# byteowlz/kokorox

Measured on AMD Instinct MI355X. Metric: real-time factor (audio-s/wall-s), 24 kHz, batch=64, higher is better.
Workload: dtype f32 in / out, f32 accumulate; products on split operands: f16f8 (a_hi b_hi on f16 MFMAs, the cross terms a_lo b_hi + a_hi b_lo of the 7 / 11-tap convs on e4m3 scaled MFMAs: ~17 significant bits per product; every other conv f16x3: ~22) -- wider than the bf16 BASELINE configs[2] names, inside the 1e-; 1 GPU; batch=64/GPU synthetic 128-phoneme utterances (T=130), durations pinned 3,3,3,4 -> F=422 frames = 10.55 s each, noise on, inputs in HBM; batch_per_gpu=64, frames=422, parallelism=utterance-sharded x1, one-time weight broadcast

## Files before the change

### kokorox_amd/build.py

```python
from __future__ import annotations

import os
import subprocess
import sys

HERE = os.path.dirname(os.path.abspath(__file__))
CSRC = os.path.join(HERE, "csrc")
LIB_DIR = os.path.join(HERE, "lib")
LIB_PATH = os.path.join(LIB_DIR, "libkokorox_hip.so")
TEST_LIB_PATH = os.path.join(LIB_DIR, "libkokorox_hip_test.so")
TEST_SOURCES = ["test_hooks.hip"]
SOURCES = ["conv_mfma.hip", "conv_f16x3.hip", "conv_f16x3_da.hip", "conv_f16x3_da_p1.hip", "conv_f16x3_da_w2.hip", "conv_f16x3_da_s16.hip", "conv_f16x3_da_f8.hip", "conv_f16x3_da_pre.hip", "conv_f16x3_pre.hip", "conv_f16x3_dapn.hip", "conv_f16x3_dag.hip", "kernels_misc.hip", "model.hip", "api.hip", "dispatcher.hip", "onnx_import.cpp"]
HEADERS = ["kx_common.h", "kx_error.h", "conv_epilogue.h", "conv_f16x3_common.h"]
_PUB = os.path.join("..", "..", "include", "kokorox_hip.h")
_PUB_TEST = os.path.join("..", "..", "include", "kokorox_hip_test.h")
EXTRA_DEPS = {"model.hip": ["onnx_import.h", "model.h", _PUB], "api.hip": ["model.h", "kx_handle.h", "api_guard.h", _PUB],
              "dispatcher.hip": ["model.h", "kx_handle.h", "dispatcher_core.h", _PUB],
              "test_hooks.hip": ["model.h", "kx_handle.h", "api_guard.h", _PUB, _PUB_TEST], "onnx_import.cpp": ["onnx_import.h"], "conv_f16x3_da_p1.hip": ["conv_f16x3_da.hip"], "conv_f16x3_da_w2.hip": ["conv_f16x3_da.hip"], "conv_f16x3_da_s16.hip": ["conv_f16x3_da.hip"], "conv_f16x3_da_f8.hip": ["conv_f16x3_da.hip"], "conv_f16x3_da_pre.hip": ["conv_f16x3_da.hip"]}
FLAGS = ["-O3", "--offload-arch=gfx950", "-fPIC", "-std=c++17", "-Wall", "-Wno-unused-result"]


def _hipcc() -> str:
    for cand in (os.environ.get("HIPCC"), "/opt/rocm/bin/hipcc", "hipcc"):
        if cand and (os.path.isabs(cand) and os.path.exists(cand) or not os.path.isabs(cand)):
            return cand
    return "hipcc"


def _newer(target: str, deps) -> bool:
    if not os.path.exists(target):
        return False
    t = os.path.getmtime(target)
    return all(os.path.getmtime(d) <= t for d in deps)


LAST_BUILD = {"compiled": [], "reused": [], "linked": False}


def build_library(force: bool = False, verbose: bool = False) -> str:
    LAST_BUILD["compiled"], LAST_BUILD["reused"], LAST_BUILD["linked"] = [], [], False
    os.makedirs(LIB_DIR, exist_ok=True)
    hdrs = [os.path.join(CSRC, h) for h in HEADERS]
    objs, test_objs, jobs = [], [], []
    for src in SOURCES + TEST_SOURCES:
        s = os.path.join(CSRC, src)
        o = os.path.join(LIB_DIR, os.path.splitext(src)[0] + ".o")
        (test_objs if src in TEST_SOURCES else objs).append(o)
        if force or not _newer(o, [s] + hdrs + [os.path.join(CSRC, d) for d in EXTRA_DEPS.get(src, [])]):
            flags = [f for f in FLAGS if not f.startswith("--offload-arch")] if src.endswith(".cpp") else FLAGS
            jobs.append([_hipcc(), *flags, "-c", s, "-o", o])
            LAST_BUILD["compiled"].append(src)
# ... 30 lines not shown
```

### kokorox_amd/csrc/conv_f16x3.hip

```cpp
#include "conv_f16x3_common.h"

namespace kx {

template <int BM, int BN, int WM, int WN, int ACT, int TK, bool PF, int VT>
__global__ __launch_bounds__(WM * WN * 64, (WM * WN == 8) ? 4 : ((BM / WM / 32) * (BN / WN / 32) > 6 ? 2 : 3))
void conv1d_f16x3_kernel(const ConvArgs a) {
    constexpr int MT = BM / WM / 32;
    constexpr int NT = BN / WN / 32;
    constexpr int NWV = WM * WN;
    static_assert((NWV == 4 || NWV == 8) && MT >= 1 && NT >= 1, "4 or 8 waves per workgroup");
    static_assert(VT == 1 || (VT <= TK && PF), "virtual taps need TK >= VT and the prefetching build");
    extern __shared__ __attribute__((aligned(16))) unsigned char smem16[];

    const int tid = threadIdx.x;
    const int lane = tid & 63;
    const int wave = __builtin_amdgcn_readfirstlane(tid >> 6);
    const int wm = wave / WN, wn = wave % WN;
    const int r = lane & 31, h = lane >> 5;
    const int b = blockIdx.z, ct = blockIdx.y;
    int tile_x = blockIdx.x;
    if (a.xcd_swizzle && gridDim.x >= 16) {
        const int nx = gridDim.x;
        const int off = (int)(((long)nx * (blockIdx.y + (long)gridDim.y * blockIdx.z)) & 7);
        const int cls = (blockIdx.x + off) & 7;
// ... 328 lines not shown

template <int BM, int BN, int WM, int WN, int ACT, int TK>
static void launch_inst16_act(const ConvArgs& a, int B, int max_cols, hipStream_t s) {
    static const int pf_env = env_int("KX_PF", 1);
    const int XW = (BN - 1) * a.stride + (a.K - 1) * a.dil + 1;
    if (pf_env && a.stride == 1 && XW <= BN + 128)
        launch_inst16_pf<BM, BN, WM, WN, ACT, TK, true>(a, B, max_cols, s);
    else
        launch_inst16_pf<BM, BN, WM, WN, ACT, TK, false>(a, B, max_cols, s);
}

template <int BM, int BN, int WM, int WN, int TK>
static void launch_inst16_tk(const ConvArgs& a, int B, int max_cols, hipStream_t s) {
    if (a.act == ACT_SNAKE)
        launch_inst16_act<BM, BN, WM, WN, ACT_SNAKE, TK>(a, B, max_cols, s);
    else if (a.act == ACT_LEAKY)
        launch_inst16_act<BM, BN, WM, WN, ACT_LEAKY, TK>(a, B, max_cols, s);
    else
        launch_inst16_act<BM, BN, WM, WN, ACT_NONE, TK>(a, B, max_cols, s);
}

template <int BM, int BN, int WM, int WN>
static void launch_inst16(const ConvArgs& a, int B, int max_cols, hipStream_t s) {
#ifndef KX_TK
#define KX_TK 3
#endif
    launch_inst16_tk<BM, BN, WM, WN, KX_TK>(a, B, max_cols, s);
}

void conv16_pick_tile(int BM, int max_cols, int B, int Cout, int K, int dil, int stride, int* bn, int* wn, int ws_force, bool stats,
                      int act, int n_chunks16, int pmode) {
    static const int force = env_int("KX_BN", 0);
    if (ws_force != 1 && act >= 0 && conv16_da_s16_shape(BM, K, dil, stride, act, n_chunks16, false, pmode)) {
        const bool small = (long)((max_cols + 255) / 256) * ((Cout + 127) / 128) * B < 256 && ws_force != 2;
        *bn = small ? 128 : 192;
        *wn = small ? 2 : 3;
        return;
    }
    if (ws_force == 2 && conv16_da_eligible(BM, K, dil, stride, 0)) {
        *bn = 256; *wn = 2;
        return;
    }
    if (BM != 128) {
        *bn = 256; *wn = 4;
    } else if ((force == 128 || max_cols <= 160) && !stats) {
        *bn = 128; *wn = 2;
    } else if ((long)((max_cols + 255) / 256) * ((Cout + 127) / 128) * B < 256 && force != 256) {
        *bn = 128; *wn = 1;
    } else {
        *bn = 256; *wn = 2;
    }
}

int conv16_flat_bn(const ConvArgs& a, int BM, int B, int max_cols) {
    static const int on = env_int("KX_FLAT", 1);
    if (!on || BM != 128 || B < 2 || max_cols <= 0 || a.merge_T > 0 || a.ws_force == 1 || a.stamps) return 0;
    if (a.K == 1 && a.stride == 1 && !a.stat_part && !a.in_up2 && a.n_chunks16 >= 3 && a.act != ACT_SNAKE) return 0;
    int bn, wn;
    conv16_pick_tile(BM, max_cols, B, a.Cout, a.K, a.dil, a.stride, &bn, &wn, a.ws_force, a.stat_part != nullptr, a.act, a.n_chunks16,
                     conv16_pmode(a));
    if (conv16_da_s16_shape(BM, a.K, a.dil, a.stride, a.act, a.n_chunks16, a.merge_T > 0, conv16_pmode(a))) return bn;
    if (bn == 128 && wn == 1) return conv16_use_da(BM, a.K, a.dil, a.stride, a.merge_T > 0) ? 128 : 0;
    if (bn == 128) return 0;
    return conv16_use_da(BM, a.K, a.dil, a.stride, a.merge_T > 0) ? 256 : 0;
}

void launch_conv1d_f16x3(const ConvArgs& a, int BM, int B, int max_cols, hipStream_t s) {
#ifdef KX_ONLY_MAIN
    launch_inst16_pf<128, 256, 2, 2, ACT_SNAKE, 3, true>(a, B, max_cols, s);
    return;
#else
    KX_REQUIRE(a.n_chunks16 == (a.Cin + CK16 - 1) / CK16 && a.w16 != nullptr, "conv1d f16x3: weights not packed");
// ... 215 lines not shown
```

### kokorox_amd/csrc/conv_f16x3_da.hip

```cpp
#include "conv_f16x3_common.h"
#include <type_traits>


#ifndef KX_F8_RAW_AUX
#define KX_F8_RAW_AUX 0
#endif
#ifndef KX_F8_HWCOS
#define KX_F8_HWCOS 1
#endif

namespace kx {

template <int I, int N, class F>
__device__ __forceinline__ void static_for(F&& f) {
    if constexpr (I < N) {
        f(std::integral_constant<int, I>{});
        static_for<I + 1, N>(f);
    }
}

#if !defined(KX_DA_P1) && !defined(KX_DA_W2) && !defined(KX_DA_S16) && !defined(KX_DA_PRE)
bool conv16_da_eligible(int BM, int K, int dil, int stride, int merged) {
    return BM == 128 && stride == 1 && !merged && (K - 1) * dil + 256 <= 384;
}
// ... 14 lines not shown
    }
    static constexpr int age(int kind, int id) {
        int n = 0, result = -1;
        int st_h[3 * KT + 8] = {}, st_x[3 * NC + 8] = {};
        for (int sc = 0; sc < 2; ++sc) {
            for (int p = 0; p < KT; ++p) {
                if (p == HS) n += RAW;
                if (sc == 1) {
                    if (kind == 0 && p == id) result = n - st_h[KT + p];
                    if (kind == 1 && cross_of(p) == id) result = n - st_x[NC + id];
                }
                n += 2;
                st_h[p + RH <= KT - 1 ? sc * KT + p + RH : (sc + 1) * KT + p % RH] = n;
                const int c = cross_of(p);
                if (c >= 0) {
                    n += 4;
                    st_x[sc * NC + c + RC] = n;
                }
            }
            n += RAW;
        }
        return result < 63 ? result : 63;
    }
    static constexpr int cum(int NB, int first, int n) {
        int t = 0;
        for (int r = 0; r < n; ++r) t += cross_of((first + r) / NB) >= 0 ? 3 : 1;
        return t;
    }
    static constexpr int hu_before(int NB, int NA, int HU, int first, int I0, int rel) {
        return rel > I0 ? ((cum(NB, first, rel) - cum(NB, first, I0)) * HU) / (cum(NB, first, NA) - cum(NB, first, I0)) : 0;
    }
};

template <int ACT, int KT, int NTT, bool P1, bool W2 = false, bool S16 = false, bool PRE = false, bool BF = false, bool F8 = false>
__global__ __launch_bounds__(256, (NTT == 8 || S16) ? 2 : 3) void conv1d_f16x3_da_kernel(const ConvArgs a) {
    static_assert(!BF || P1, "BF: a form of the reduced-precision kernels only");
    static_assert(!F8 || (S16 && KT % 4 == 3), "F8: a form of the S16 loop; tap groups of four with one padding slot");
    constexpr bool HWC = F8 && KX_F8_HWCOS;
    static_assert(!PRE || (!P1 && !S16 && ACT == ACT_NONE), "PRE: the activation lives in the image; f16x3 forms on 32x32x16 only");
    static_assert(!W2 || (KT >= 3 && (KT & 1) && NTT == 8), "W2: odd compile-time tap counts on the 256-column tile");
    static_assert(!S16 || (KT >= 3 && (KT & 1) && !P1 && !W2), "S16: odd compile-time tap counts, three MFMAs per product, 4 x 1 waves");
    static_assert(NTT == 8 || NTT == 4 || (NTT == 6 && S16), "tile widths: 256, 128, and 192 columns in the S16 form");
    constexpr int BM = 128, NT = NTT, BN = 32 * NT;
    constexpr bool W64 = KT > 0;
    constexpr bool SPLIT = W64 && BN % 128 == 0;
    constexpr int NJF = W64 ? (SPLIT ? BN / 128 : (BN + 64) / 128) : (BN + 128) / 128;
    constexpr int NJ = NJF + (SPLIT ? 1 : 0);
    constexpr int HU = 8 * NJF + (SPLIT ? 4 : 0);
    constexpr int XWp = W64 ? BN + 64 : BN + 128;
    static_assert(!W64 || SPLIT || (BN + 64) % 128 == 0, "the window is whole 64-column blocks in pairs, or ends in a split block");
    constexpr int XBUF = 4 * XWp;
    constexpr int tap_units = 4 * BM;
    extern __shared__ __attribute__((aligned(16))) unsigned char smem16[];
    uint4* Xs = reinterpret_cast<uint4*>(smem16);

    const int tid = threadIdx.x;
    const int lane = tid & 63;
    const int wave = __builtin_amdgcn_readfirstlane(tid >> 6);
    const int r = lane & 31, h = lane >> 5;
    auto pack_pair = [](float v0, float v1, unsigned& hi_pk, unsigned& lo_pk) __attribute__((always_inline)) {
        if constexpr (BF) {
            auto rne = [](float x) __attribute__((always_inline)) {
                unsigned u = __builtin_bit_cast(unsigned, x);
                u += 0x7fffu + ((u >> 16) & 1u);
                return u >> 16;
            };
            hi_pk = rne(v0) | (rne(v1) << 16);
            lo_pk = 0u;
        } else if constexpr (F8) {
            split_pair_f8(v0, v1, hi_pk, lo_pk);
        } else {
            split_pair(v0, v1, hi_pk, lo_pk);
        }
    };
    auto act_in = [](float y, float slope, float al, float ial) __attribute__((always_inline)) {
        if constexpr (ACT == ACT_SNAKE && HWC) {
            const float u = (al * y) * 0.318309886183790672f;
            return __builtin_fmaf(ial, __builtin_fmaf(-0.5f, __builtin_amdgcn_cosf(u), 0.5f), y);
        } else {
// ... 22 lines not shown
            const int mid = (lo + hi) >> 1;
            if (a.tile_prefix[mid] <= gt) lo = mid;
            else hi = mid;
        }
        b = __builtin_amdgcn_readfirstlane(lo);
        tile_x = gt - a.tile_prefix[b];
    } else {
        const int nx = gridDim.x, ny = gridDim.y, N = nx * ny;
        const int l = blockIdx.x + nx * blockIdx.y;
        int lp = l;
        if (a.xcd_swizzle && N >= 16) {
            const int off = (int)(((long)N * blockIdx.z) & 7);
            const int cls = (l + off) & 7;
            int start = 0;
            for (int c = 0; c < cls; ++c) {
                const int first = (c - off) & 7;
                start += first < N ? (N - first + 7) >> 3 : 0;
            }
            lp = start + (l >> 3);
        }
        if (a.xcd_swizzle) {
            tile_x = lp / ny;
            ct = lp - tile_x * ny;
        }
    }
    if (a.dephase_cycles > 0) {
        const unsigned gl = blockIdx.x + gridDim.x * (blockIdx.y + gridDim.y * blockIdx.z);
        const bool late = a.dephase_mode == 1 ? (gl < 512u && ((gl >> 3) & 1u)) : (gl >= 256u && gl < 512u);
        if (late) {
            const unsigned long long t_end = __builtin_amdgcn_s_memtime() + (unsigned long long)a.dephase_cycles;
            while (__builtin_amdgcn_s_memtime() < t_end) __builtin_amdgcn_s_sleep(64);
        }
    }
    const int t0 = tile_x * BN;
    const int Lin = a.in_len.lens[b] * a.in_len.mul + a.in_len.add;
    const int Lout = a.out_len.lens[b] * a.out_len.mul + a.out_len.add;
    const int ncols = (a.store == ST_UPSCATTER) ? (Lin + 1) : Lout;
    if (t0 >= ncols) return;

    const int K = KT > 0 ? KT : a.K, dil = a.dil;
    const int n_chunks = a.n_chunks16;
    const int n_steps = n_chunks * K;
    const float* xb = a.x + (long)b * a.x_bs;
    const int p0 = t0 - a.pad;
    const bool has_norm = a.nmean != nullptr;
    const int up2 = a.in_up2;
    const int Lsrc = up2 ? ((Lin + 1) >> 1) : Lin;

    f32x16 acc[1][NT];
#pragma unroll
    for (int j = 0; j < NT; ++j)
#pragma unroll
        for (int e = 0; e < 16; ++e) acc[0][j][e] = 0.f;
    constexpr int NB16 = S16 ? 2 * NT : 1;
    f32x4v acc16[2][NB16];
#pragma unroll
    for (int i = 0; i < 2; ++i)
#pragma unroll
        for (int j = 0; j < NB16; ++j) acc16[i][j] = f32x4v{0.f, 0.f, 0.f, 0.f};

    const int g = wave & 1, jb = wave >> 1;
    float raw[NJ][8];
    float praw[4];
    int xoff[NJ];
    unsigned okmask = 0;
    auto blk_col = [&](int j) __attribute__((always_inline)) { return (SPLIT && j == NJF) ? 64 * 2 * NJF : 64 * (jb + 2 * j); };
#pragma unroll
    for (int j = 0; j < NJ; ++j) {
        const int p = p0 + lane + blk_col(j);
        okmask |= (p >= 0 && p < Lin) ? (1u << j) : 0u;
        int pi = up2 ? (p >> 1) : p;
        pi = pi < 0 ? 0 : (pi >= Lsrc ? Lsrc - 1 : pi);
        xoff[j] = pi;
    }
    using u32x4 = __attribute__((ext_vector_type(4))) unsigned;
    constexpr int NLD = PRE ? (4 * XWp) / 256 : 1;
    static_assert(!PRE || (4 * XWp) % 256 == 0, "PRE: whole rounds of 256 lanes");
    u32x4 rawq[NLD];
    unsigned qoff[NLD];
    unsigned okq = 0;
    const buf_rsrc xq = make_buf(PRE ? reinterpret_cast<const char*>(a.x16) + (long)b * a.x16_bs : reinterpret_cast<const char*>(a.x));
    const unsigned chunk_bytes = PRE ? 64u * (unsigned)a.x16_ld : 0u;
    const buf_rsrc xrow = make_buf(xb);
    if constexpr (PRE) {
#pragma unroll
        for (int i = 0; i < NLD; ++i) {
            const int idx = tid + 256 * i, plane = idx / XWp, u = idx - plane * XWp;
            const int p = p0 + u;
            okq |= (p >= 0 && p < Lin) ? (1u << i) : 0u;
            const int pc = p < 0 ? 0 : (p >= Lin ? Lin - 1 : p);
            qoff[i] = 16u * (unsigned)(plane * a.x16_ld + pc);
        }
    }
    const int cmax_in = a.Cin - 1;
    const float* nm_src = has_norm ? a.nmean + (long)b * a.n_bs : xb;
    const float* ns_src = has_norm ? a.nscale + (long)b * a.n_bs : xb;
    const float* nh_src = has_norm ? a.nshift + (long)b * a.n_bs : xb;
    auto load_params = [&](int ch, float (&pv)[4]) __attribute__((always_inline)) {
        const int c = ch * CK16 + g * 8 + (lane & 7);
// ... 290 lines not shown
#define F8_WAIT_T1 if (a.stamps) acc_wait += __builtin_amdgcn_s_memrealtime() - tb0;
#else
#define F8_BAR_T0
#define F8_BAR_T1
#define F8_WAIT_T1
#endif
#ifndef KX_F8_RH
#define KX_F8_RH ((KT - 1) % 3 != 0 ? 3 : 4)
#endif
#ifndef KX_F8_RC
#define KX_F8_RC (NT == 6 ? 1 : 2)
#endif
        constexpr int RH = KX_F8_RH, RC = KX_F8_RC;
        using FS = F8Sched<KT, RH, RC, raw_ops>;
        constexpr int NG = FS::NG, NC = FS::NC;
        static_assert(RH <= KT && (KT - 1) % RH != 0 && NC % RC == 0, "f16f8: static ring slots");
        static_assert(2 * (NG - 1) <= HS && KT - 1 - 2 * (NG - 1) >= HS && (HS & 1), "f16f8: cross groups inside their buffer's phase");
        const int n_super = n_chunks >> 1;
        const int d_norm = tau16 ? dil : 0, d_str = tau16 ? XBUF - (KT - 1) * dil : 0;
        int d_x2 = tau16 ? 2 * dil : 0;
        int d_xl = tau16 ? 0 : dil;
        using v8i = __attribute__((ext_vector_type(8))) int;
        u32x4 hs[RH][2], xs[RC][4];
        auto make_srd = [](const void* base) __attribute__((always_inline)) {
            const unsigned long long pa = (unsigned long long)base;
            u32x4 srd;
            srd[0] = __builtin_amdgcn_readfirstlane((unsigned)pa);
            srd[1] = __builtin_amdgcn_readfirstlane((unsigned)(pa >> 32) & 0xffffu);
            srd[2] = 0xffffffffu;
            srd[3] = 0x00020000u;
            return srd;
        };
        const u32x4 srd_h = make_srd(a.w16), srd_x = make_srd(a.w8x);
        const unsigned voff_h = 16u * (unsigned)(tau16 * tap_units + h16 * BM + wave * 32 + r16);
        const unsigned voff_x = 16u * (unsigned)((lane >> 4) * 256 + wave * 32 + r16);
        const unsigned tile_h = (unsigned)__builtin_amdgcn_readfirstlane(ct * n_steps), tile_x8 = (unsigned)__builtin_amdgcn_readfirstlane(ct * n_chunks * NG);
        auto load_H = [&](int s0, u32x4 (&xh)[2]) __attribute__((always_inline)) {
            const unsigned so = (tile_h + (unsigned)__builtin_amdgcn_readfirstlane(s0 < n_steps - 2 ? s0 : n_steps - 2)) * (16u * tap_units);
            asm volatile("buffer_load_dwordx4 %0, %1, %2, %3 offen" : "=v"(xh[0]) : "v"(voff_h), "s"(srd_h), "s"(so) : "memory");
            asm volatile("buffer_load_dwordx4 %0, %1, %2, %3 offen offset:256" : "=v"(xh[1]) : "v"(voff_h), "s"(srd_h), "s"(so) : "memory");
        };
        auto load_X = [&](int chunk, const int m, u32x4 (&x)[4]) __attribute__((always_inline)) {
            const unsigned so = (tile_x8 + (unsigned)__builtin_amdgcn_readfirstlane(chunk < n_chunks ? chunk : n_chunks - 1) * NG + m) * 16384u;
            asm volatile("buffer_load_dwordx4 %0, %1, %2, %3 offen" : "=v"(x[0]) : "v"(voff_x), "s"(srd_x), "s"(so) : "memory");
            asm volatile("buffer_load_dwordx4 %0, %1, %2, %3 offen offset:2048" : "=v"(x[1]) : "v"(voff_x), "s"(srd_x), "s"(so) : "memory");
            asm volatile("buffer_load_dwordx4 %0, %1, %2, %3 offen offset:256" : "=v"(x[2]) : "v"(voff_x), "s"(srd_x), "s"(so) : "memory");
            asm volatile("buffer_load_dwordx4 %0, %1, %2, %3 offen offset:2304" : "=v"(x[3]) : "v"(voff_x), "s"(srd_x), "s"(so) : "memory");
        };
        static_for<0, RH>([&](auto qc) __attribute__((always_inline)) { load_H(2 * decltype(qc)::value, hs[decltype(qc)::value]); });
        static_for<0, RC>([&](auto qc) __attribute__((always_inline)) {
            constexpr int c = decltype(qc)::value;
            load_X(c >= NG ? 1 : 0, c >= NG ? c - NG : c, xs[c]);
        });
        asm volatile("s_waitcnt vmcnt(0)" ::: "memory");
        int xl_it = h16 * XWp + r16;
        int dil_it = dil;
        half8 fh[2];
        v8i fx[2];
        auto load_blk_h = [&](const int p, const int nb, half8& fhx) __attribute__((always_inline)) {
            const int f0 = 2 * p, b0 = f0 >= KT ? 1 : 0, tp = f0 - b0 * KT;
            const uint4* xt = Xs + (xl_it + b0 * XBUF + tp * dil_it + (f0 == KT - 1 ? d_str : d_norm) + nb * 16);
            fhx = *reinterpret_cast<const half8*>(xt);
        };
        auto load_blk_x = [&](const int c, const int nb, v8i& fxx) __attribute__((always_inline)) {
            const int b0 = c >= NG ? 1 : 0, m = c - b0 * NG;
            const uint4* xt = Xs + (xl_it + 2 * XWp + b0 * XBUF + 4 * m * dil_it + d_x2 + nb * 16);
            const uint4 u0 = *xt, u1 = *(xt + (m == NG - 1 ? d_xl : dil_it));
            fxx = v8i{(int)u0.x, (int)u0.y, (int)u0.z, (int)u0.w, (int)u1.x, (int)u1.y, (int)u1.z, (int)u1.w};
        };
// ... 550 lines not shown
                        for (int c = 0; c < 8; ++c) asm volatile("" ::"v"(raw[j][c]));
                } else if (!(a.dbg & 1))
                    stage_from_raw(Xs + (cur ^ 1) * XBUF, ch);
                asm volatile("s_waitcnt lgkmcnt(0)\n\ts_barrier" ::: "memory");
                cur ^= 1;
                if (ch + 1 < n_chunks && !(a.dbg & (1 | 2048))) {
                    load_raw(ch + 1);
                    age += raw_ops;
                    o1 += raw_ops;
                    o2 += raw_ops;
                }
                load_tile(0, 0, fh[(E0 + NT) % 3], fl[(E0 + NT) % 3]);
                load_tile(0, 1, fh[(E0 + NT + 1) % 3], fl[(E0 + NT + 1) % 3]);
            }
        }
    };
    for (int s3 = 0; s3 < n_steps; s3 += 3) {
        step(0, ah0, al0, age0, age1, age2, s3);
        if (s3 + 1 < n_steps) step(NT % 3, ah1, al1, age1, age2, age0, s3 + 1);
        if (s3 + 2 < n_steps) step((2 * NT) % 3, ah2, al2, age2, age0, age1, s3 + 2);
    }
    }
    asm volatile("s_waitcnt vmcnt(0)" ::: "memory");
#ifdef KX_DA_STAMPS
    if (a.stamps) st2 = __builtin_amdgcn_s_memrealtime();
#endif
    if (a.dbg & 8) return;
    asm volatile("s_waitcnt lgkmcnt(0)\n\ts_barrier" ::: "memory");
    float2* stat_scr = reinterpret_cast<float2*>(smem16) + wave * (32 * 33);
    float* wide_scr = reinterpret_cast<float*>(stat_scr);
    if constexpr (S16) {
        static_for<0, NT / 2>([&](auto gc) __attribute__((always_inline)) {
            constexpr int g2 = decltype(gc)::value;
            conv_store_group16<EPI_ROWS, NB16, 2, NT == 6>(a, acc16, 4 * g2, a.w_unscale, b, ct * BM + wave * 32, t0 + 64 * g2, lane, ncols, Lout,
                                                  tile_x * (NT / 2) + g2, stat_scr, wide_scr);
        });
    } else if constexpr (W2) {
        conv_store_group<EPI_ROWS, true>(a, *reinterpret_cast<f32x16(*)[1][4]>(&acc[0][0]), a.w_unscale, b, ct * BM + wr2 * 64, t0 + 128 * wc2, r,
                                   h, ncols, Lout, tile_x * 2 + wc2, stat_scr, wide_scr);
        conv_store_group<EPI_ROWS, true>(a, *reinterpret_cast<f32x16(*)[1][4]>(&acc[0][4]), a.w_unscale, b, ct * BM + wr2 * 64 + 32, t0 + 128 * wc2,
                                   r, h, ncols, Lout, tile_x * 2 + wc2, stat_scr, wide_scr);
    } else if constexpr (NT == 8) {
        conv_store_group<EPI_ROWS>(a, *reinterpret_cast<f32x16(*)[1][4]>(&acc[0][0]), a.w_unscale, b, ct * BM + wave * 32, t0, r, h,
                                   ncols, Lout, tile_x * 2, stat_scr, wide_scr);
        conv_store_group<EPI_ROWS>(a, *reinterpret_cast<f32x16(*)[1][4]>(&acc[0][4]), a.w_unscale, b, ct * BM + wave * 32, t0 + 128, r,
                                   h, ncols, Lout, tile_x * 2 + 1, stat_scr, wide_scr);
    } else {
        conv_store_group<EPI_ROWS>(a, acc, a.w_unscale, b, ct * BM + wave * 32, t0, r, h, ncols, Lout, tile_x, stat_scr, wide_scr);
    }
#ifdef KX_DA_STAMPS
    if (a.stamps && tid == 0) {
        const unsigned lin = blockIdx.x + gridDim.x * (blockIdx.y + gridDim.y * blockIdx.z);
        unsigned long long* o = a.stamps + (unsigned long long)lin * 8;
        o[0] = st0; o[1] = st1; o[2] = st2;
        __builtin_amdgcn_s_waitcnt(0);
        o[3] = __builtin_amdgcn_s_memrealtime();
        o[4] = __builtin_amdgcn_s_getreg(63492);
        o[5] = __builtin_readcyclecounter() - cyc0;
        o[6] = F8 ? acc_wait : __builtin_amdgcn_s_getreg(63508);
        o[7] = acc_bar;
    }
#endif
}

#ifdef KX_DA_P1
constexpr bool DA_P1 = true;
#else
constexpr bool DA_P1 = false;
#endif

#ifdef KX_DA_W2
constexpr bool DA_W2 = true;
#else
constexpr bool DA_W2 = false;
#endif

#ifdef KX_DA_S16
constexpr bool DA_S16 = true;
#else
constexpr bool DA_S16 = false;
#endif

#ifdef KX_DA_F8
constexpr bool DA_F8 = true;
#else
constexpr bool DA_F8 = false;
#endif

template <int ACT, int KT, int NTT, bool W2X = DA_W2, bool PREX = false, bool BFX = false>
static void launch_da_inst(const ConvArgs& a, int B, int max_cols, hipStream_t s) {
    auto kern = conv1d_f16x3_da_kernel<ACT, KT, NTT, DA_P1, W2X, DA_S16, PREX, BFX, DA_F8>;
    constexpr int BN = 32 * NTT;
    constexpr size_t lds_x = 16 * (size_t)2 * 4 * (BN + 128), lds_scr = 4 * 32 * 33 * sizeof(float2);
    constexpr size_t lds = lds_x > lds_scr ? lds_x : lds_scr;
    dim3 grid((max_cols + BN - 1) / BN, (a.Cout + 127) / 128, B);
    KX_REQUIRE(grid.x > 0 && grid.y > 0 && grid.y < 65536 && B > 0 && B < 65536, "conv1d f16x3 da: bad grid");
    if (a.tile_prefix) {
        KX_REQUIRE(a.flat_ny == (int)grid.y && a.flat_B == B && a.flat_bn_host == BN && a.flat_tiles_host > 0 &&
                       (long)a.flat_tiles_host * grid.y < (1L << 30),
                   "conv1d f16x3 da: flat tile list does not match the launch");
        grid = dim3((unsigned)a.flat_tiles_host * grid.y, 1, 1);
    }
    hipLaunchKernelGGL(kern, grid, dim3(256), lds, s, a);
    KX_HIP(hipGetLastError());
}

#ifdef KX_DA_PRE
void launch_conv1d_f16x3_da_pre(const ConvArgs& a, int B, int max_cols, hipStream_t s, int bn) {
    KX_REQUIRE(a.x16 != nullptr && a.x16_ld > 0 && !a.in_up2 && !a.prec1 && a.stride == 1 && a.merge_T == 0,
               "conv1d f16x3 da pre: launch not eligible");
    KX_REQUIRE(bn == 256 || bn == 128, "conv1d f16x3 da pre: tile of 256 or 128 columns");
    KX_REQUIRE((long)a.n_chunks16 * 64 * a.x16_ld < (1L << 31), "conv1d f16x3 da pre: image of one utterance beyond 2 GiB");
    if (bn == 128 && conv16_dapn_eligible(a)) {
        launch_conv1d_f16x3_dapn(a, B, max_cols, s);
        return;
    }
    const bool w64 = a.K == 3 && (a.K - 1) * a.dil <= 64;
    if (bn == 256) {
        if (w64) launch_da_inst<ACT_NONE, 3, 8, true, true>(a, B, max_cols, s);
        else launch_da_inst<ACT_NONE, 0, 8, false, true>(a, B, max_cols, s);
    } else {
        if (w64) launch_da_inst<ACT_NONE, 3, 4, false, true>(a, B, max_cols, s);
        else launch_da_inst<ACT_NONE, 0, 4, false, true>(a, B, max_cols, s);
    }
}
#elif defined(KX_DA_F8)
static bool f8_k3() {
    static const int on = getenv("KX_F8_K3") ? atoi(getenv("KX_F8_K3")) : 1;
    return on != 0;
}
bool conv16_da_f8_shape(int K, int dil) { return (K == 11 || K == 7 || (K == 3 && f8_k3())) && (K - 1) * dil <= 64; }
void launch_conv1d_f16x3_da_f8(const ConvArgs& a, int B, int max_cols, hipStream_t s, int bn) {
    KX_REQUIRE(a.w8x != nullptr && conv16_da_f8_shape(a.K, a.dil) && a.act == ACT_SNAKE && a.stride == 1 && a.merge_T == 0 && !a.prec1 &&
                   a.n_chunks16 >= 2 && (a.n_chunks16 & 1) == 0,
               "conv1d f16x3 da f8: launch not eligible");
    KX_REQUIRE(bn == 192 || bn == 128, "conv1d f16x3 da f8: tile of 192 or 128 columns");
    KX_REQUIRE((long)a.Cin * a.x_ld * 4 < (1L << 32), "conv1d f16x3 da f8: input tensor of one utterance beyond 4 GiB");
    if (a.K == 11) {
        if (bn == 192) launch_da_inst<ACT_SNAKE, 11, 6>(a, B, max_cols, s);
        else launch_da_inst<ACT_SNAKE, 11, 4>(a, B, max_cols, s);
// ... 75 lines not shown

#if defined(KX_DA_W2) || defined(KX_DA_S16) || defined(KX_DA_PRE)
#elif defined(KX_DA_P1)
void launch_conv1d_f16x3_da_p1(const ConvArgs& a, int B, int max_cols, hipStream_t s, int bn) {
    if (a.prec1 == 2) {
        KX_REQUIRE(a.w16b != nullptr, "conv1d f16x3 da p1: no bf16 weight image");
        ConvArgs b16 = a;
        b16.w16 = a.w16b;
        if (bn == 256) launch_da_ntt<8, true>(b16, B, max_cols, s);
        else launch_da_ntt<4, true>(b16, B, max_cols, s);
        return;
    }
    if (bn == 256)
        launch_da_ntt<8>(a, B, max_cols, s);
    else
        launch_da_ntt<4>(a, B, max_cols, s);
}
#else
void launch_conv1d_f16x3_da_p1(const ConvArgs& a, int B, int max_cols, hipStream_t s, int bn);
void launch_conv1d_f16x3_da_pre(const ConvArgs& a, int B, int max_cols, hipStream_t s, int bn);

void launch_conv1d_f16x3_da(const ConvArgs& a, int B, int max_cols, hipStream_t s, int bn) {
    KX_REQUIRE(conv16_da_eligible(128, a.K, a.dil, a.stride, a.merge_T > 0), "conv1d f16x3 da: launch not eligible");
    KX_REQUIRE(a.n_chunks16 == (a.Cin + CK16 - 1) / CK16 && a.w16 != nullptr, "conv1d f16x3 da: weights not packed");
    KX_REQUIRE(a.epi != EPI_GELU_NEW, "conv1d f16x3 da: no gelu epilogue");
    KX_REQUIRE(bn == 256 || bn == 128 || bn == 192, "conv1d f16x3 da: tile of 256, 192 or 128 columns");
    if (max_cols <= 0) return;
    if (a.x16) {
        KX_REQUIRE(bn != 192, "conv1d f16x3 da: no pre-split form of the 192-column tile");
        launch_conv1d_f16x3_da_pre(a, B, max_cols, s, bn);
        return;
    }
    if (conv16_da_s16_shape(128, a.K, a.dil, a.stride, a.act, a.n_chunks16, a.merge_T > 0, conv16_pmode(a))) {
        if (a.w8x && conv16_da_f8_shape(a.K, a.dil)) launch_conv1d_f16x3_da_f8(a, B, max_cols, s, bn == 128 ? 128 : 192);
        else launch_conv1d_f16x3_da_s16(a, B, max_cols, s, bn == 128 ? 128 : 192);
        return;
    }
    KX_REQUIRE(bn != 192, "conv1d f16x3 da: the 192-column tile exists in the S16 form only");
    if (a.prec1) {
        launch_conv1d_f16x3_da_p1(a, B, max_cols, s, bn);
        return;
    }
    static const int dephase = getenv("KX_DEPHASE") ? atoi(getenv("KX_DEPHASE")) : 0;
    static const int dephase_mode = getenv("KX_DEPHASE_MODE") ? atoi(getenv("KX_DEPHASE_MODE")) : 1;
    if (dephase > 0 && bn == 256) {
        ConvArgs d = a;
        const long grid_n = (long)((max_cols + 255) / 256) * ((a.Cout + 127) / 128) * B;
        const double tile_cycles = (double)a.n_chunks16 * a.K * 8 * 96 * 2.5 + 50000.0;
        d.dephase_cycles = grid_n >= 1024 ? (int)(tile_cycles * dephase / 1000.0) : 0;
        d.dephase_mode = dephase_mode;
        launch_da_ntt<8>(d, B, max_cols, s);
        return;
    }
    if (bn == 256)
        launch_da_ntt<8>(a, B, max_cols, s);
    else
        launch_da_ntt<4>(a, B, max_cols, s);
}
#endif

}
```

### kokorox_amd/csrc/kx_common.h

```cpp
#pragma once
#include <hip/hip_runtime.h>

#include <cmath>
#include <cstdint>
#include <cstring>
#include <cstdio>
#include <stdexcept>
#include <string>

#include <atomic>
#include <mutex>

#include "kx_error.h"

namespace kx {

constexpr int KX_MAX_DEVICES = 64;

struct DynLdsLimit {
    std::atomic<size_t> limit[KX_MAX_DEVICES];
    std::mutex mu;
    DynLdsLimit() {
        for (auto& l : limit) l.store(64 * 1024);
    }
// ... 110 lines not shown

struct PackSrc {
    const float* p[3];
    int rows[3];
};
void launch_pack_conv(const PackSrc& src, float* dst, int Cout, int Cin, int K, int BM, hipStream_t s);
void launch_pack_convT(const float* w, float* dst, int Cin, int Cout, int s, int BM, hipStream_t s_);
size_t packed_conv_floats(int rows, int Cin, int K, int BM);

enum ConvMode { CONV_F32 = 0, CONV_F16X3 = 1, CONV_F16X3_LDS = 2, CONV_F16X3_DA = 3, CONV_F16 = 4, CONV_BF16 = 5, CONV_F16F8 = 6 };
void launch_conv1d_f16x3(const ConvArgs& a, int BM, int B, int max_cols, hipStream_t s);
inline int conv16_pmode(const ConvArgs& a) { return a.prec1 ? 1 : (a.w8x ? 2 : 0); }
void conv16_pick_tile(int BM, int max_cols, int B, int Cout, int K, int dil, int stride, int* bn, int* wn,
                      int ws_force = 0, bool stats = false, int act = -1, int n_chunks16 = 0, int pmode = 0);
bool conv16_use_da(int BM, int K, int dil, int stride, int merged);
bool conv16_da_eligible(int BM, int K, int dil, int stride, int merged);
void launch_conv1d_f16x3_da(const ConvArgs& a, int B, int max_cols, hipStream_t s, int bn = 256);
bool conv16_use_dag(const ConvArgs& a, int BM);
bool conv16_dag_eligible(const ConvArgs& a, int BM);
void launch_conv1d_f16x3_dag(const ConvArgs& a, int B, int max_cols, hipStream_t s);
int conv16_cu_count();
int cu_count_override();
bool conv16_da_s16_shape(int BM, int K, int dil, int stride, int act, int n_chunks16, bool merged, int pmode);
size_t packed_conv16_halves(int rows, int Cin, int K, int BM);
float device_absmax(const float* p, long n, hipStream_t s);
int pick_weight_shift(float absmax);
void launch_pack_conv16(const PackSrc& src, void* dst, int Cout, int Cin, int K, int BM, float wscale, hipStream_t s);
void launch_pack_convT16(const float* w, void* dst, int Cin, int Cout, int sd, int BM, float wscale, hipStream_t s);
void launch_image_to_bf16(const void* w16, void* dst, size_t n_halves, hipStream_t s);
size_t packed_conv8x_bytes(int rows, int Cin, int K);
void launch_pack_conv8x(const void* w16, void* dst, int rows, int Cin, int K, hipStream_t s);
bool conv16_da_f8_shape(int K, int dil);
void launch_conv1d_f16x3_da_f8(const ConvArgs& a, int B, int max_cols, hipStream_t s, int bn);

void launch_vec_add(const float* a, const float* b, float* out, int n, hipStream_t s);
void launch_transpose_whh(const float* whh, float* out, hipStream_t s);

void launch_albert_embed(const int64_t* ids, long ids_stride, const float* word, const float* type0,
                         const float* pos, float* out, long bs, int ld, const int* lens, int B, int Tmax,
                         int n_vocab, unsigned* bad_id, hipStream_t s);
void launch_embed(const int64_t* ids, long ids_stride, const float* table, int C, float* out, long bs, int ld,
                  const int* lens, int B, int Tmax, int n_vocab, unsigned* bad_id, hipStream_t s);

enum LnMode { LN_PLAIN = 0, LN_AFFINE = 1, LN_ADA = 2 };
void launch_layernorm_ch(const float* x, float* y, long bs, int ld, int C, LenMap len, int B, int Lmax,
                         float eps, int mode, const float* g, const float* be, int g_bs, float leaky,
                         hipStream_t s);

void launch_attention(const float* qkv, long bs, int ld, float* ctx, long cbs, int cld, const int* lens, int B,
                      int Tmax, hipStream_t s);

struct FcDesc {
    const float* w;
    const float* b;
    int n_out;
    int style_off;
    long out_off;
};
void launch_style_fc(const FcDesc* d_desc, int n_desc, const float* styles, float* out, long out_bs, int B,
                     hipStream_t s);

void launch_stats_finalize(const float2* part, int tiles, int cols_per_tile, int C, LenMap len, int B, const float* gb,
                           long gb_bs, float* mean, float* scale, float* shift, int n_bs, hipStream_t s);
void launch_in_stats(const float* x, long bs, int ld, int C, LenMap len, int B, const float* gb, long gb_bs,
                     float* mean, float* scale, float* shift, int n_bs, float2* raw_out, hipStream_t s);

// ... 46 lines not shown
```

### kokorox_amd/csrc/model.hip

```cpp
#include <chrono>
#include "model.h"

#include <sys/stat.h>
#include <unistd.h>

#include <cstdlib>
#include <cstring>

#include "onnx_import.h"

namespace kx {

static constexpr float RSQRT2 = 0.70710678118654752f;
static inline int up4(int x) { return (x + 31) & ~31; }

static thread_local int tl_cu_override = 0;
int cu_count_override() { return tl_cu_override; }
struct CuScope {
    int saved;
    explicit CuScope(int n) : saved(tl_cu_override) { tl_cu_override = n; }
    ~CuScope() { tl_cu_override = saved; }
};

Model::Model(int dev, int part, int n_parts) : device(dev), part_(part), n_parts_(n_parts) {
// ... 593 lines not shown
    parts_.erase(out.p);
    static const bool fuse_stats = !(getenv("KX_FUSE_STATS") && atoi(getenv("KX_FUSE_STATS")) == 0);
    if (fuse_stats && o.stat_part && o.store == ST_NORMAL && !o.accum) {
        const int max_c = out.Lmax;
        int bn, wn;
        if (f16) {
            conv16_pick_tile(w.BM, max_c, B_, w.rows, w.K, o.dil, o.stride, &bn, &wn, 0, true, o.act, w.n_chunks16, conv16_pmode(a));
        } else {
            bn = conv_bn(w.BM);
            wn = w.BM == 128 ? 2 : 4;
        }
        a.stat_part = o.stat_part;
        a.stat_tiles = ((max_c + bn - 1) / bn) * wn;
        parts_[out.p] = PartInfo{o.stat_part, a.stat_tiles, bn / wn, w.rows};
    }
    static const int dbg_env = getenv("KX_DBG") ? atoi(getenv("KX_DBG")) : 0;
    a.dbg = dbg_env;
    int max_cols = (o.store == ST_UPSCATTER) ? in.Lmax + 1 : out.Lmax;
    static const bool merge_env = !(getenv("KX_MERGE") && atoi(getenv("KX_MERGE")) == 0);
    if (merge_env && f16 && B_ > 1 && w.K == 1 && o.stride == 1 && o.pad == 0 && !o.in_up2 && !o.nmean &&
        o.store != ST_UPSCATTER && !o.stat_part && in.Lmax <= 512 && in.len.mul == 1 && in.len.add == 0 &&
        out.len.lens == in.len.lens && out.len.mul == 1 && out.len.add == 0) {
        a.merge_T = in.Lmax;
        a.merge_B = B_;
        max_cols = B_ * in.Lmax;
    }
    if (f16 && B_ > 1) {
        const int fbn = conv16_flat_bn(a, w.BM, B_, max_cols);
        if (fbn) {
            const LenMap& lm = (o.store == ST_UPSCATTER) ? a.in_len : a.out_len;
            const int extra = o.store == ST_UPSCATTER ? 1 : 0;
            int total = 0;
            a.tile_prefix = tile_prefix_for(lm, extra, fbn, &total);
            a.flat_ny = (w.rows + 127) / 128;
            a.flat_B = B_;
            a.flat_tiles_host = total;
            a.flat_bn_host = fbn;
            if (total <= 0) return;
        }
    }
    static const char* stamp_path = getenv("KX_STAMP");
    static bool stamped = false;
    unsigned long long* d_stamps = nullptr;
    long n_wg = 0;
    static const int stamp_rows = getenv("KX_STAMP_ROWS") ? atoi(getenv("KX_STAMP_ROWS")) : 128;
    static const int stamp_k = getenv("KX_STAMP_K") ? atoi(getenv("KX_STAMP_K")) : 11;
    static int stamp_skip = getenv("KX_STAMP_SKIP") ? atoi(getenv("KX_STAMP_SKIP")) : 0;
    const bool stamp_match = stamp_path && !stamped && f16 && w.K == stamp_k && w.rows == stamp_rows && B_ >= 8 && !dry_;
    if (stamp_match && stamp_skip > 0) --stamp_skip;
    else if (stamp_match) {
        n_wg = (long)((max_cols + 127) / 128) * ((w.rows + 127) / 128) * (a.merge_T > 0 ? 1 : B_);
        KX_HIP(hipMalloc((void**)&d_stamps, n_wg * 64));
        KX_HIP(hipMemsetAsync(d_stamps, 0, n_wg * 64, stream_));
        a.stamps = d_stamps;
    }
    if (x16_bs) {
        launch_split_image(a, B_, in.Lmax, x16, x16_bs, stream_);
        a.x16 = x16;
        a.x16_bs = x16_bs;
        a.x16_ld = in.ld;
    }
    if (prof_on_ && w.BM == 128) {
        const LenMap& lm = (o.store == ST_UPSCATTER) ? in.len : out.len;
        const std::vector<int>& hl = (lm.lens == dT_) ? hT_ : hF_;
        double cols = 0;
        for (int b = 0; b < B_; ++b) cols += (double)hl[b] * lm.mul + lm.add + (o.store == ST_UPSCATTER ? 1 : 0);
        prof_flops_ += 2.0 * w.rows * w.Cin * w.K * cols;
// ... 1194 lines not shown
```

### kokorox_amd/hip_koko.py

```python
from __future__ import annotations

import ctypes as C
import os
from typing import List, Optional, Sequence

import numpy as np

_HERE = os.path.dirname(os.path.abspath(__file__))
LIB_PATH = os.path.join(_HERE, "lib", "libkokorox_hip.so")

PACK_F32_MONO, PACK_F32_STEREO, PACK_PCM16_MONO = 0, 1, 2
KX_OK, KX_ERR_INVALID, KX_ERR_IO, KX_ERR_DEVICE, KX_ERR_STATE = 0, 1, 2, 3, 4
KX_FLAG_NOISE_OFF = 1
KX_FLAG_TAPS = 2
STYLE_DIM = 256
SAMPLES_PER_FRAME = 600

_lib = None


class KokoroxHipError(RuntimeError):
    def __init__(self, code: int, msg: str):
        super().__init__(f"kokorox_hip error {code}: {msg}")
        self.code = code
# ... 490 lines not shown
        return {"requests": a.value, "batches": b.value, "max_batch": c.value, "batches_per_model": list(per),
                "replayed_requests": rp.value, "retried_batches": rt.value, "healthy": [int(v) for v in hl],
                "failed_models": mf.value, "requeued_requests": rq.value}

    def close(self):
        if getattr(self, "_d", None):
            self._lib.kx_dispatcher_destroy(self._d)
            self._d = None

    def __del__(self):
        try:
            self.close()
        except Exception:
            pass


def import_onnx(onnx_path: str, out_path: str) -> str:
    lib = load_library()
    err = C.create_string_buffer(2048)
    rc = lib.kx_import_onnx(os.fsencode(onnx_path), os.fsencode(out_path), err, len(err))
    if rc != KX_OK:
        raise KokoroxHipError(rc, err.value.decode(errors="replace"))
    return out_path


def _err_call(fn, *args):
    err = C.create_string_buffer(512)
    rc = fn(*args, err, len(err))
    if rc != 0:
        raise KokoroxHipError(rc, err.value.decode())


CONV_F32, CONV_F16X3, CONV_F16F8 = 0, 1, 6
STFT_ONNX, STFT_TORCH = 0, 1


def conv1d(x, w, bias=None, stride=1, pad=0, dil=1, transposed=False, act=0, slope=0.0, alpha=None, norm=None,
           device=0, mode=None, pre=False):
    lib = load_test_library()
    if mode is None:
        mode = CONV_F32 if os.environ.get("KOKOROX_CONV", "") == "f32" else CONV_F16X3
    x, w = _f32(x), _f32(w)
    B, Cin, L = x.shape
    k = w.shape[2]
    if transposed:
        Cout = w.shape[1]
        Lout = (L - 1) * stride - 2 * pad + k
    else:
        Cout = w.shape[0]
        Lout = (L + 2 * pad - dil * (k - 1) - 1) // stride + 1
    y = np.zeros((B, Cout, Lout), dtype=np.float32)
    bias, alpha, norm = _f32(bias), _f32(alpha), _f32(norm)
    _err_call(lib.kx_test_conv1d, device, _ptr(x), B, Cin, L, _ptr(w), _ptr(bias), Cout, k, stride, pad, dil,
              1 if transposed else 0, act, float(slope), _ptr(alpha), _ptr(norm), _ptr(y), Lout, mode | (0x100 if pre else 0))
    return y


def conv_transpose(x, w, bias=None, stride=6, act=1, slope=0.1, resid=None, up_off=0, mode=1, pre=False, device=0):
    lib = load_test_library()
    x, w = _f32(x), _f32(w)
    B, Cin, L = x.shape
    Cout, k = w.shape[1], w.shape[2]
    assert k == 2 * stride
    pad = (k - stride) // 2
    Lout = (L - 1) * stride - 2 * pad + k
    y = np.zeros((B, Cout, Lout + (1 if up_off else 0)), dtype=np.float32)
# ... 66 lines not shown
```

Measured before the change: 6952 x realtime.

## Add 256-row eight-wave variant of the f16f8 snake conv kernel

Adds a compiled variant of the direct-access f16f8 conv kernel that uses 512 threads (8 waves) covering 256 output rows per workgroup instead of 128. Each pair of 4-wave halves shares the staged input tile, so input columns are loaded into LDS once for twice as many output channels. It is selected by default for 256-channel snake convs with K=3/7/11, a 192-column tile and no residual or accumulate, and the flat tile grid is resized to match. In exchange it runs at one workgroup per CU by launch bounds and may need more than 64 KiB of LDS, which lowers occupancy and latency hiding.

```diff
diff --git a/kokorox_amd/build.py b/kokorox_amd/build.py
--- a/kokorox_amd/build.py
+++ b/kokorox_amd/build.py
@@ -10,13 +10,13 @@
 LIB_PATH = os.path.join(LIB_DIR, "libkokorox_hip.so")
 TEST_LIB_PATH = os.path.join(LIB_DIR, "libkokorox_hip_test.so")
 TEST_SOURCES = ["test_hooks.hip"]
-SOURCES = ["conv_mfma.hip", "conv_f16x3.hip", "conv_f16x3_da.hip", "conv_f16x3_da_p1.hip", "conv_f16x3_da_w2.hip", "conv_f16x3_da_s16.hip", "conv_f16x3_da_f8.hip", "conv_f16x3_da_pre.hip", "conv_f16x3_pre.hip", "conv_f16x3_dapn.hip", "conv_f16x3_dag.hip", "kernels_misc.hip", "model.hip", "api.hip", "dispatcher.hip", "onnx_import.cpp"]
+SOURCES = ["conv_mfma.hip", "conv_f16x3.hip", "conv_f16x3_da.hip", "conv_f16x3_da_p1.hip", "conv_f16x3_da_w2.hip", "conv_f16x3_da_s16.hip", "conv_f16x3_da_f8.hip", "conv_f16x3_da_f8w.hip", "conv_f16x3_da_pre.hip", "conv_f16x3_pre.hip", "conv_f16x3_dapn.hip", "conv_f16x3_dag.hip", "kernels_misc.hip", "model.hip", "api.hip", "dispatcher.hip", "onnx_import.cpp"]
 HEADERS = ["kx_common.h", "kx_error.h", "conv_epilogue.h", "conv_f16x3_common.h"]
 _PUB = os.path.join("..", "..", "include", "kokorox_hip.h")
 _PUB_TEST = os.path.join("..", "..", "include", "kokorox_hip_test.h")
 EXTRA_DEPS = {"model.hip": ["onnx_import.h", "model.h", _PUB], "api.hip": ["model.h", "kx_handle.h", "api_guard.h", _PUB],
               "dispatcher.hip": ["model.h", "kx_handle.h", "dispatcher_core.h", _PUB],
-              "test_hooks.hip": ["model.h", "kx_handle.h", "api_guard.h", _PUB, _PUB_TEST], "onnx_import.cpp": ["onnx_import.h"], "conv_f16x3_da_p1.hip": ["conv_f16x3_da.hip"], "conv_f16x3_da_w2.hip": ["conv_f16x3_da.hip"], "conv_f16x3_da_s16.hip": ["conv_f16x3_da.hip"], "conv_f16x3_da_f8.hip": ["conv_f16x3_da.hip"], "conv_f16x3_da_pre.hip": ["conv_f16x3_da.hip"]}
+              "test_hooks.hip": ["model.h", "kx_handle.h", "api_guard.h", _PUB, _PUB_TEST], "onnx_import.cpp": ["onnx_import.h"], "conv_f16x3_da_p1.hip": ["conv_f16x3_da.hip"], "conv_f16x3_da_w2.hip": ["conv_f16x3_da.hip"], "conv_f16x3_da_s16.hip": ["conv_f16x3_da.hip"], "conv_f16x3_da_f8.hip": ["conv_f16x3_da.hip"], "conv_f16x3_da_f8w.hip": ["conv_f16x3_da.hip"], "conv_f16x3_da_pre.hip": ["conv_f16x3_da.hip"]}
 FLAGS = ["-O3", "--offload-arch=gfx950", "-fPIC", "-std=c++17", "-Wall", "-Wno-unused-result"]
 
 
diff --git a/kokorox_amd/csrc/conv_f16x3.hip b/kokorox_amd/csrc/conv_f16x3.hip
--- a/kokorox_amd/csrc/conv_f16x3.hip
+++ b/kokorox_amd/csrc/conv_f16x3.hip
@@ -384,12 +384,12 @@
                       int act, int n_chunks16, int pmode) {
     static const int force = env_int("KX_BN", 0);
     if (ws_force != 1 && act >= 0 && conv16_da_s16_shape(BM, K, dil, stride, act, n_chunks16, false, pmode)) {
-        const bool small = (long)((max_cols + 255) / 256) * ((Cout + 127) / 128) * B < 256 && ws_force != 2;
+        const bool small = (long)((max_cols + 255) / 256) * ((Cout + 127) / 128) * B < 256 && ws_force < 2;
         *bn = small ? 128 : 192;
         *wn = small ? 2 : 3;
         return;
     }
-    if (ws_force == 2 && conv16_da_eligible(BM, K, dil, stride, 0)) {
+    if (ws_force >= 2 && conv16_da_eligible(BM, K, dil, stride, 0)) {
         *bn = 256; *wn = 2;
         return;
     }
diff --git a/kokorox_amd/csrc/conv_f16x3_da.hip b/kokorox_amd/csrc/conv_f16x3_da.hip
--- a/kokorox_amd/csrc/conv_f16x3_da.hip
+++ b/kokorox_amd/csrc/conv_f16x3_da.hip
@@ -70,8 +70,20 @@
     }
 };
 
+#ifdef KX_DA_R256
+#define KX_DA_KERNEL_NAME conv1d_f16x3_da_r256_kernel
+#define KX_DA_BOUNDS(NTT, S16) __launch_bounds__(512, 1)
+constexpr int DA_NW = 8;
+#else
+#define KX_DA_KERNEL_NAME conv1d_f16x3_da_kernel
+#define KX_DA_BOUNDS(NTT, S16) __launch_bounds__(256, ((NTT) == 8 || (S16)) ? 2 : 3)
+constexpr int DA_NW = 4;
+#endif
+
 template <int ACT, int KT, int NTT, bool P1, bool W2 = false, bool S16 = false, bool PRE = false, bool BF = false, bool F8 = false>
-__global__ __launch_bounds__(256, (NTT == 8 || S16) ? 2 : 3) void conv1d_f16x3_da_kernel(const ConvArgs a) {
+__global__ KX_DA_BOUNDS(NTT, S16) void KX_DA_KERNEL_NAME(const ConvArgs a) {
+    constexpr int NW = DA_NW, NWP = NW / 2;
+    static_assert(NW == 4 || (F8 && NTT == 6), "R256: the f16f8 form's 192-column tile only");
     static_assert(!BF || P1, "BF: a form of the reduced-precision kernels only");
     static_assert(!F8 || (S16 && KT % 4 == 3), "F8: a form of the S16 loop; tap groups of four with one padding slot");
     constexpr bool HWC = F8 && KX_F8_HWCOS;
@@ -82,7 +94,8 @@
     constexpr int BM = 128, NT = NTT, BN = 32 * NT;
     constexpr bool W64 = KT > 0;
     constexpr bool SPLIT = W64 && BN % 128 == 0;
-    constexpr int NJF = W64 ? (SPLIT ? BN / 128 : (BN + 64) / 128) : (BN + 128) / 128;
+    static_assert(NW == 4 || (W64 && !SPLIT && (BN + 64) % (64 * NWP) == 0), "R256: whole 64-column blocks, one per wave pair");
+    constexpr int NJF = W64 ? (SPLIT ? BN / 128 : (BN + 64) / (64 * NWP)) : (BN + 128) / 128;
     constexpr int NJ = NJF + (SPLIT ? 1 : 0);
     constexpr int HU = 8 * NJF + (SPLIT ? 4 : 0);
     constexpr int XWp = W64 ? BN + 64 : BN + 128;
@@ -171,6 +184,7 @@
             while (__builtin_amdgcn_s_memtime() < t_end) __builtin_amdgcn_s_sleep(64);
         }
     }
+    const int ctw = 2 * ct + (wave >> 2), wq = wave & 3;
     const int t0 = tile_x * BN;
     const int Lin = a.in_len.lens[b] * a.in_len.mul + a.in_len.add;
     const int Lout = a.out_len.lens[b] * a.out_len.mul + a.out_len.add;
@@ -203,7 +217,7 @@
     float praw[4];
     int xoff[NJ];
     unsigned okmask = 0;
-    auto blk_col = [&](int j) __attribute__((always_inline)) { return (SPLIT && j == NJF) ? 64 * 2 * NJF : 64 * (jb + 2 * j); };
+    auto blk_col = [&](int j) __attribute__((always_inline)) { return (SPLIT && j == NJF) ? 64 * 2 * NJF : 64 * (jb + NWP * j); };
 #pragma unroll
     for (int j = 0; j < NJ; ++j) {
         const int p = p0 + lane + blk_col(j);
@@ -560,9 +574,10 @@
             return srd;
         };
         const u32x4 srd_h = make_srd(a.w16), srd_x = make_srd(a.w8x);
-        const unsigned voff_h = 16u * (unsigned)(tau16 * tap_units + h16 * BM + wave * 32 + r16);
-        const unsigned voff_x = 16u * (unsigned)((lane >> 4) * 256 + wave * 32 + r16);
-        const unsigned tile_h = (unsigned)__builtin_amdgcn_readfirstlane(ct * n_steps), tile_x8 = (unsigned)__builtin_amdgcn_readfirstlane(ct * n_chunks * NG);
+        const unsigned voff_h = 16u * (unsigned)(tau16 * tap_units + h16 * BM + (NW == 8 ? wq : wave) * 32 + r16);
+        const unsigned voff_x = 16u * (unsigned)((lane >> 4) * 256 + (NW == 8 ? wq : wave) * 32 + r16);
+        const unsigned tile_h = (unsigned)__builtin_amdgcn_readfirstlane((NW == 8 ? ctw : ct) * n_steps),
+                       tile_x8 = (unsigned)__builtin_amdgcn_readfirstlane((NW == 8 ? ctw : ct) * n_chunks * NG);
         auto load_H = [&](int s0, u32x4 (&xh)[2]) __attribute__((always_inline)) {
             const unsigned so = (tile_h + (unsigned)__builtin_amdgcn_readfirstlane(s0 < n_steps - 2 ? s0 : n_steps - 2)) * (16u * tap_units);
             asm volatile("buffer_load_dwordx4 %0, %1, %2, %3 offen" : "=v"(xh[0]) : "v"(voff_h), "s"(srd_h), "s"(so) : "memory");
@@ -1179,7 +1194,7 @@
     if constexpr (S16) {
         static_for<0, NT / 2>([&](auto gc) __attribute__((always_inline)) {
             constexpr int g2 = decltype(gc)::value;
-            conv_store_group16<EPI_ROWS, NB16, 2, NT == 6>(a, acc16, 4 * g2, a.w_unscale, b, ct * BM + wave * 32, t0 + 64 * g2, lane, ncols, Lout,
+            conv_store_group16<EPI_ROWS, NB16, 2, NT == 6>(a, acc16, 4 * g2, a.w_unscale, b, NW == 8 ? ctw * BM + wq * 32 : ct * BM + wave * 32, t0 + 64 * g2, lane, ncols, Lout,
                                                   tile_x * (NT / 2) + g2, stat_scr, wide_scr);
         });
     } else if constexpr (W2) {
@@ -1236,11 +1251,15 @@
 
 template <int ACT, int KT, int NTT, bool W2X = DA_W2, bool PREX = false, bool BFX = false>
 static void launch_da_inst(const ConvArgs& a, int B, int max_cols, hipStream_t s) {
-    auto kern = conv1d_f16x3_da_kernel<ACT, KT, NTT, DA_P1, W2X, DA_S16, PREX, BFX, DA_F8>;
-    constexpr int BN = 32 * NTT;
-    constexpr size_t lds_x = 16 * (size_t)2 * 4 * (BN + 128), lds_scr = 4 * 32 * 33 * sizeof(float2);
+    auto kern = KX_DA_KERNEL_NAME<ACT, KT, NTT, DA_P1, W2X, DA_S16, PREX, BFX, DA_F8>;
+    constexpr int BN = 32 * NTT, WG_ROWS = 32 * DA_NW;
+    constexpr size_t lds_x = 16 * (size_t)2 * 4 * (BN + 128), lds_scr = DA_NW * 32 * 33 * sizeof(float2);
     constexpr size_t lds = lds_x > lds_scr ? lds_x : lds_scr;
-    dim3 grid((max_cols + BN - 1) / BN, (a.Cout + 127) / 128, B);
+    if constexpr (lds > 64 * 1024) {
+        static DynLdsLimit lds_limit;
+        lds_limit.ensure(reinterpret_cast<const void*>(kern), lds);
+    }
+    dim3 grid((max_cols + BN - 1) / BN, (a.Cout + WG_ROWS - 1) / WG_ROWS, B);
     KX_REQUIRE(grid.x > 0 && grid.y > 0 && grid.y < 65536 && B > 0 && B < 65536, "conv1d f16x3 da: bad grid");
     if (a.tile_prefix) {
         KX_REQUIRE(a.flat_ny == (int)grid.y && a.flat_B == B && a.flat_bn_host == BN && a.flat_tiles_host > 0 &&
@@ -1248,11 +1267,26 @@
                    "conv1d f16x3 da: flat tile list does not match the launch");
         grid = dim3((unsigned)a.flat_tiles_host * grid.y, 1, 1);
     }
-    hipLaunchKernelGGL(kern, grid, dim3(256), lds, s, a);
+    hipLaunchKernelGGL(kern, grid, dim3(64 * DA_NW), lds, s, a);
     KX_HIP(hipGetLastError());
 }
 
-#ifdef KX_DA_PRE
+#ifdef KX_DA_R256
+bool conv16_da_f8w_use(const ConvArgs& a, int bn) {
+    static const int on = getenv("KX_F8_R256") ? atoi(getenv("KX_F8_R256")) : 1;
+    const bool want = a.ws_force == 3 || (a.ws_force == 0 && (on == 2 || (on == 1 && a.resid == nullptr && !a.accum)));
+    return want && bn == 192 && a.w8x != nullptr && a.Cout == 256 && a.act == ACT_SNAKE && a.stride == 1 && a.merge_T == 0 && !a.prec1 &&
+           (a.K == 3 || a.K == 7 || a.K == 11) && conv16_da_f8_shape(a.K, a.dil) && a.n_chunks16 >= 2 && (a.n_chunks16 & 1) == 0;
+}
+int conv16_da_wg_rows(const ConvArgs& a, int bn) { return conv16_da_f8w_use(a, bn) ? 256 : 128; }
+void launch_conv1d_f16x3_da_f8w(const ConvArgs& a, int B, int max_cols, hipStream_t s) {
+    KX_REQUIRE(conv16_da_f8w_use(a, 192), "conv1d f16x3 da f8w: launch not eligible");
+    KX_REQUIRE((long)a.Cin * a.x_ld * 4 < (1L << 32), "conv1d f16x3 da f8w: input tensor of one utterance beyond 4 GiB");
+    if (a.K == 11) launch_da_inst<ACT_SNAKE, 11, 6>(a, B, max_cols, s);
+    else if (a.K == 7) launch_da_inst<ACT_SNAKE, 7, 6>(a, B, max_cols, s);
+    else launch_da_inst<ACT_SNAKE, 3, 6>(a, B, max_cols, s);
+}
+#elif defined(KX_DA_PRE)
 void launch_conv1d_f16x3_da_pre(const ConvArgs& a, int B, int max_cols, hipStream_t s, int bn) {
     KX_REQUIRE(a.x16 != nullptr && a.x16_ld > 0 && !a.in_up2 && !a.prec1 && a.stride == 1 && a.merge_T == 0,
                "conv1d f16x3 da pre: launch not eligible");
@@ -1394,7 +1428,8 @@
         return;
     }
     if (conv16_da_s16_shape(128, a.K, a.dil, a.stride, a.act, a.n_chunks16, a.merge_T > 0, conv16_pmode(a))) {
-        if (a.w8x && conv16_da_f8_shape(a.K, a.dil)) launch_conv1d_f16x3_da_f8(a, B, max_cols, s, bn == 128 ? 128 : 192);
+        if (a.w8x && conv16_da_f8_shape(a.K, a.dil) && bn != 128 && conv16_da_f8w_use(a, 192)) launch_conv1d_f16x3_da_f8w(a, B, max_cols, s);
+        else if (a.w8x && conv16_da_f8_shape(a.K, a.dil)) launch_conv1d_f16x3_da_f8(a, B, max_cols, s, bn == 128 ? 128 : 192);
         else launch_conv1d_f16x3_da_s16(a, B, max_cols, s, bn == 128 ? 128 : 192);
         return;
     }
diff --git a/kokorox_amd/csrc/conv_f16x3_da_f8w.hip b/kokorox_amd/csrc/conv_f16x3_da_f8w.hip
--- /dev/null
+++ b/kokorox_amd/csrc/conv_f16x3_da_f8w.hip
@@ -0,0 +1,4 @@
+#define KX_DA_S16 1
+#define KX_DA_F8 1
+#define KX_DA_R256 1
+#include "conv_f16x3_da.hip"
diff --git a/kokorox_amd/csrc/kx_common.h b/kokorox_amd/csrc/kx_common.h
--- a/kokorox_amd/csrc/kx_common.h
+++ b/kokorox_amd/csrc/kx_common.h
@@ -166,6 +166,9 @@
 void launch_pack_conv8x(const void* w16, void* dst, int rows, int Cin, int K, hipStream_t s);
 bool conv16_da_f8_shape(int K, int dil);
 void launch_conv1d_f16x3_da_f8(const ConvArgs& a, int B, int max_cols, hipStream_t s, int bn);
+bool conv16_da_f8w_use(const ConvArgs& a, int bn);
+int conv16_da_wg_rows(const ConvArgs& a, int bn);
+void launch_conv1d_f16x3_da_f8w(const ConvArgs& a, int B, int max_cols, hipStream_t s);
 
 void launch_vec_add(const float* a, const float* b, float* out, int n, hipStream_t s);
 void launch_transpose_whh(const float* whh, float* out, hipStream_t s);
diff --git a/kokorox_amd/csrc/model.hip b/kokorox_amd/csrc/model.hip
--- a/kokorox_amd/csrc/model.hip
+++ b/kokorox_amd/csrc/model.hip
@@ -649,7 +649,8 @@
             const int extra = o.store == ST_UPSCATTER ? 1 : 0;
             int total = 0;
             a.tile_prefix = tile_prefix_for(lm, extra, fbn, &total);
-            a.flat_ny = (w.rows + 127) / 128;
+            const int wg_rows = conv16_da_wg_rows(a, fbn);
+            a.flat_ny = (w.rows + wg_rows - 1) / wg_rows;
             a.flat_B = B_;
             a.flat_tiles_host = total;
             a.flat_bn_host = fbn;
diff --git a/kokorox_amd/hip_koko.py b/kokorox_amd/hip_koko.py
--- a/kokorox_amd/hip_koko.py
+++ b/kokorox_amd/hip_koko.py
@@ -546,6 +546,7 @@
 
 
 CONV_F32, CONV_F16X3, CONV_F16F8 = 0, 1, 6
+HOOK_F8, HOOK_F8_R256, HOOK_EPI_STREAM = 0x200, 0x400, 0x800
 STFT_ONNX, STFT_TORCH = 0, 1
 
 
```

Result: no change. 6986 x realtime (median of 6 runs) (+0.5%).
